# wwhitecyan/satellite-pose-estimation

Measured on AMD Instinct MI355X. Metric: images/sec end-to-end (backbone->kpts->PnP) at 416x416; SPEED pose score, higher is better.
Workload: dtype bf16; 1 GPU; BASELINE config 2: ResNet50-s8 + 6/6 DETR, 11 queries, 416x416, solver=epnp; global_batch=64, per_gpu_batch=64, input_size=416, num_queries=11, attention_dtype=bf16 q/k, fp16 V/P, parallelism=dp1 (image sharding)

## Files before the change

include/spe.h:

```cpp
#ifndef SPE_H_
#define SPE_H_
#include <stdint.h>

#ifdef __cplusplus
extern "C" {
#endif

#define SPE_ABI_VERSION 9

enum {
  SPE_E_ARG = -1,
  SPE_E_STATE = -2,
  SPE_E_MISSING = -3,
  SPE_E_KEY = -4,
  SPE_E_WORKSPACE = -5,
  SPE_E_LAUNCH = -6
};

enum { SPE_DTYPE_BF16_ = 0, SPE_DTYPE_F32_ = 1, SPE_DTYPE_F16_ = 2, SPE_DTYPE_F32X3_ = 4, SPE_DTYPE_F32X6_ = 5,
       SPE_DTYPE_F32H3_ = 6 };

enum { SPE_PNP_EPNP = 0, SPE_PNP_RANSAC_P3P_LM = 1, SPE_PNP_EPNP_RANSAC_SIGMA = 2, SPE_PNP_EPNP_LM = 3,
       SPE_PNP_EPNP_CERES = 4, SPE_PNP_EXHAUSTIVE = 5 };

// ... 153 lines not shown
                   int W, int Cin, int KH, int KW, int stride, int pad, const void* Bw, int ldb, int M, int N, int K,
                   const float* bias, const void* R, int ldr, int act_code, void* C, int ldc, int out_f32, int vt_T,
                   int vt_B, int r_period, const float* ln_g, const float* ln_b, int out_f16);
int spe_debug_gemm_path(void);
int spe_debug_gemm_h3(void* stream, int mode, const void* A, int lda, int H, int W, int Cin, int KH, int KW, int stride,
                      int pad, int ldb, int M, int N, int K, const float* bias, const void* R, int ldr, int act_code,
                      void* C, int ldc, const void* planes, int plane_rows, const float* sinv, const float* amax_a,
                      float* amax_c, float amax_c_mul);
int spe_debug_ffn_h3(void* stream, const float* x, int ldx, float* y, int ldy, int M, int F, const void* w1, int ld1,
                     const float* meta1, const void* w2, int ld2, const float* sinv2, const float* b2,
                     const float* gamma, const float* beta, const float* amax_x, float sh);
int spe_debug_ffn_h3_perm(int p);
int spe_debug_gemm_planes(void* stream, int dtype, int mode, const void* A, int lda, const void* P, int ldp, int prow,
                          int H, int W, int Cin, int KH, int KW, int stride, int pad, const void* Bw, int ldb, int M,
                          int N, int K, const float* bias, const void* R, int ldr, int act_code, void* C, int ldc,
                          const void* planes, int plane_rows);
int spe_debug_attention(void* stream, int dtype, const void* q, int ldq, const void* k, int ldk, const void* vt,
                        void* o, int ldo, int B, int H, int Tq, int Tk, float scale);
int spe_debug_attn_map(void* stream, const void* q, const void* k, int B, int H, int Tq, int Tk, int dtype, float* out);
int spe_debug_layernorm(void* stream, int dtype, const void* x, const float* gamma, const float* beta, void* out,
                        float* out_f32, int M, int D);
int spe_debug_ffn(void* stream, const void* x, int ldx, const void* w1, int ld1, const float* b1, const void* w2,
                  int ld2, const float* b2, const float* gamma, const float* beta, void* y, int ldy, int M, int D,
                  int F, float* partial, int splits);
int spe_debug_xattn(void* stream, const void* q, int ldq, const void* k, int ldk, const void* v, int ldv, void* u,
                    int ldu, const void* wv, const float* bv, void* o, int ldo, int B, int Q, int T, int splits,
                    float* partial_scratch);
int spe_debug_xattn_h3(void* stream, const float* q, int ldq, const float* mem, const float* pos, const float* mem_amax,
                       const float* wv, const float* bv, float* o, int ldo, float* o_amax, int B, int Q, int T,
                       int splits, float* partial_scratch, void* plane_scratch);
int spe_debug_upconv(void* stream, int dtype, const void* z, void* out, int ldo, int B, int H, int W, int C);
int spe_debug_btail(void* stream, const void* a, int lda, int k1, const void* r, const void* w3, int ld3,
                    const float* b3, void* y, const void* w1p, int ld1, const float* b1, void* z, int n2, int M);
int spe_debug_decsa(void* stream, void* tgt, int ldt, int B, int Q, const void* wqk, int ldqk, const float* bqk,
                    const void* wv, int ldv, const float* bv, const void* qpos, const void* wo, int ldo,
                    const float* bo, const float* g, const float* b, float scale);
int spe_debug_decproj(void* stream, void* tgt, int ldt, const void* x, int ldx, int B, int Q, const void* wo, int ldo,
                      const float* bo, const float* g, const float* b);
int spe_debug_decxproj(void* stream, void* tgt, int ldt, float* partial_scratch, int splits, int T, int B, int Q,
                       const void* wv, int ldwv, const float* bv, const void* wo, int ldo, const float* bo,
                       const float* g, const float* b);
int spe_debug_wfrag_pack(void* stream, const void* w, int ld, int N, void* dst);
int spe_debug_decffn(void* stream, const void* x, int ldx, int M, int F, const void* w1, int ld1, const float* b1,
                     const void* w2, int ld2, const float* b2, const float* gamma, const float* beta, void* y, int ldy,
                     float* partial);
int spe_debug_decq(void* stream, const void* x, int ldx, int M, int N, const void* w, int ldw, const float* bias,
                   const void* r, int ldr, int period, void* y, int ldy);
int spe_debug_btail_perm(int k);
int spe_debug_stempool(void* stream, const void* x, const void* w, int ldw, const float* bias, void* out, int ldo,
                       int B, int S);

int spe_debug_dwconv_tiles(int Ho, int Wo);
int spe_debug_dwconv(void* stream, int dtype, const void* x, const float* w, const float* bias, void* y,
                     float* pool_partials, int B, int H, int W, int C, int k, int stride, int act);
int spe_debug_se_gate(void* stream, const float* pool_partials, int tiles, float inv_hw, const float* w1, const float* b1,
                      const float* w2t, float* scale, int B, int C, int hidden);
int spe_debug_pwconv(void* stream, int dtype, const void* a, int lda, const void* w, int ldw, const float* bias,
                     const float* scale, int rows_per_image, const void* r, int ldr, void* c, int ldc, int M, int N,
                     int K, int act);
int spe_debug_rtdetr_backbone(spe_model* m, void* stream, const float* images, int batch, void* workspace,
                              int64_t workspace_bytes, float* f0, float* f1, float* f2);

int spe_debug_ghost_cheap(void* stream, int dtype, const void* x1, int ldx, int xoff, const float* w, const float* bias,
                          void* y, const void* gate, const void* resid, float* pool_partials, int B, int H, int W,
                          int half, int act, int post);
int spe_debug_dfc_gate(void* stream, int dtype, const void* x, const float* w1, const float* b1, const float* w2,
                       const float* b2, void* gate, int B, int H, int W, int C);
int spe_debug_se_gate_bias(void* stream, const float* pool_partials, int tiles, float inv_hw, const float* w1,
                           const float* b1, const float* w2t, const float* b2, float* scale, int B, int C, int hidden);
int spe_debug_pool2(void* stream, int dtype, const void* x, void* y, int B, int H, int W, int C);

int spe_debug_rt_resample2x(void* stream, int dtype, const void* in, int ldi, void* out, int ldo, int B, int H, int W,
                            int C, int mode);
int spe_debug_rt_query_select(void* stream, int dtype, const float* logits, int C, const void* memory, int ldm,
                              const float* anchors, int B, int Q, int D, int levels, const int* lvl_start, int* topk,
                              void* target, int ldt, float* sel_logits, float* sel_anchors);
int spe_debug_rt_qpos_hidden(void* stream, int dtype, const float* ref, const float* w0, const float* b0, void* out,
                             int rows, int H);
int spe_debug_rt_head_finish(void* stream, int dtype, int rows, int Q, int C, const float* hs, const float* cls_w,
                             const float* cls_b, const void* h2, int ld_h2, const float* box_w2, const float* box_b2,
                             const float* sig_w2, const float* sig_b2, const float* pt_add, int pt_add_invsig,
// ... 11 lines not shown
```

satellite-pose-estimation_amd/csrc/debug_capi.cpp:

```cpp
#include <hip/hip_runtime.h>

#include <cmath>

#include "../../include/spe.h"
#include "model_state.h"

namespace {
thread_local const void* g_planes = nullptr;
thread_local int g_plane_rows = 0;
}

extern "C" {

int spe_debug_gemm(void* stream, int dtype, int mode, const void* A, int lda, const void* P, int ldp, int prow,
                   int H, int W, int Cin, int KH, int KW, int stride, int pad, const void* Bw, int ldb, int M, int N,
                   int K, const float* bias, const void* R, int ldr, int act_code, void* C, int ldc, int out_f32, int vt_T,
                   int vt_B, int r_period, const float* ln_g, const float* ln_b, int out_f16) {
  GemmArgs g{};
  g.A = A; g.lda = lda; g.P = P; g.ldp = ldp; g.prow = prow;
  g.H = H; g.W = W; g.Cin = Cin; g.KH = KH; g.KW = KW; g.stride = stride; g.pad = pad;
  g.Ho = mode == GEMM_CONV ? (H + 2 * pad - KH) / stride + 1 : 0;
  g.Wo = mode == GEMM_CONV ? (W + 2 * pad - KW) / stride + 1 : 0;
  g.B = Bw; g.ldb = ldb; g.M = M; g.N = N; g.K = K;
  g.bias = bias; g.R = R; g.ldr = ldr; g.act = act_code & 255; g.res_post = (act_code >> 8) & 1; g.C = C; g.ldc = ldc; g.out_f32 = out_f32;
// ... 132 lines not shown
int spe_debug_xattn_h3(void* stream, const float* q, int ldq, const float* mem, const float* pos, const float* mem_amax,
                       const float* wv, const float* bv, float* o, int ldo, float* o_amax, int B, int Q, int T,
                       int splits, float* partial_scratch, void* plane_scratch) {
  if (!q || !mem || !pos || !mem_amax || !wv || !bv || !o || !partial_scratch || !plane_scratch || B < 0 || Q < 1 ||
      T < 1)
    return spe_fail(SPE_E_ARG, "bad argument");
  hipStream_t s = (hipStream_t)stream;
  char* kp = (char*)plane_scratch;
  char* vp = kp + (size_t)B * T * 1024;
  if (spe_launch_xattn_h3_split(mem, pos, mem_amax, kp, vp, B, T, s) != 0)
    return spe_fail(SPE_E_LAUNCH, "xattn_h3 split launch failed");
  XattnArgs a{};
  a.q = q; a.ldq = ldq; a.k = kp; a.ldk = 512; a.v = vp; a.ldv = 512;
  a.wv = wv; a.bv = bv; a.o = o; a.ldo = ldo;
  a.B = B; a.Q = Q; a.T = T; a.splits = splits > 0 ? splits : spe_xattn_splits(B, Q, T);
  const size_t rows = (size_t)a.splits * B * 8 * Q;
  a.pm = partial_scratch; a.pl = partial_scratch + rows; a.pu = partial_scratch + 2 * rows;
  a.mem_amax = mem_amax; a.o_amax = o_amax;
  const int rc = spe_launch_xattn_h3(a, s);
  return rc != 0 ? spe_fail(SPE_E_LAUNCH, "xattn_h3 launch rejected its arguments") : 0;
}

int spe_debug_btail(void* stream, const void* a, int lda, int k1, const void* r, const void* w3, int ld3,
                    const float* b3, void* y, const void* w1p, int ld1, const float* b1, void* z, int n2, int M) {
  if (!a || !w3 || !b3 || !y || !w1p || !b1 || !z || M < 0) return spe_fail(SPE_E_ARG, "bad argument");
  BtailArgs t{};
  t.A = a; t.lda = lda; t.k1 = k1; t.R = r; t.ldr = 256;
  t.w3 = w3; t.ld3 = ld3; t.b3 = b3; t.y = y; t.ldy = 256; t.n1 = 256;
  t.w1 = w1p; t.ld1 = ld1; t.b1 = b1; t.z = z; t.ldz = n2; t.n2 = n2; t.M = M;
  const int rc = spe_launch_btail(t, (hipStream_t)stream);
  return rc != 0 ? spe_fail(SPE_E_LAUNCH, "btail launch rejected its arguments") : 0;
}

namespace {
struct Frags {
  std::vector<void*> bufs;
  hipStream_t s;
  int err = 0;
  explicit Frags(hipStream_t st) : s(st) {}
  const void* get(const void* w, int ld, int N) {
    if (ld == 0 || !w) return w;
    void* p = nullptr;
    if (hipMalloc(&p, (size_t)N * 256 * 2) != hipSuccess) { err = 1; return nullptr; }
    bufs.push_back(p);
    if (spe_launch_wfrag_pack(w, ld, N, p, s) != 0) err = 1;
    return p;
  }
  ~Frags() {
    if (bufs.empty()) return;
    (void)hipStreamSynchronize(s);
    for (void* p : bufs) (void)hipFree(p);
  }
};
}

int spe_debug_wfrag_pack(void* stream, const void* w, int ld, int N, void* dst) {
  const int rc = spe_launch_wfrag_pack(w, ld, N, dst, (hipStream_t)stream);
  return rc != 0 ? spe_fail(SPE_E_ARG, "wfrag_pack: bad argument") : 0;
}

int spe_debug_decsa(void* stream, void* tgt, int ldt, int B, int Q, const void* wqk, int ldqk, const float* bqk,
                    const void* wv, int ldv, const float* bv, const void* qpos, const void* wo, int ldo,
                    const float* bo, const float* g, const float* b, float scale) {
  Frags f((hipStream_t)stream);
  DecSaArgs a{};
  a.tgt = tgt; a.ldt = ldt; a.B = B; a.Q = Q;
// ... 44 lines not shown
    a.w2 = w2;
  } else {
    void* p = nullptr;
    if (hipMalloc(&p, (size_t)256 * F * 2) != hipSuccess) return spe_fail(SPE_E_ARG, "decffn: scratch");
    f.bufs.push_back(p);
    for (int c0 = 0; c0 < F; c0 += 256)
      if (spe_launch_wfrag_pack((const char*)w2 + (size_t)c0 * 2, ld2, 256, (char*)p + (size_t)c0 * 256 * 2,
                                (hipStream_t)stream))
        f.err = 1;
    a.w2 = p;
  }
  if (f.err) return spe_fail(SPE_E_ARG, "decffn: weight packing failed");
  FfnArgs r{};
  r.x = x; r.ldx = ldx; r.y = y; r.ldy = ldy; r.M = M; r.D = 256; r.F = F;
  r.b2 = b2; r.gamma = gamma; r.beta = beta; r.splits = F / 256; r.partial = partial;
  int rc = spe_launch_decffn(a, (hipStream_t)stream);
  if (!rc) rc = spe_launch_ffn_reduce_ln(r, (hipStream_t)stream);
  return rc != 0 ? spe_fail(SPE_E_LAUNCH, "decffn launch rejected its arguments") : 0;
}

int spe_debug_decq(void* stream, const void* x, int ldx, int M, int N, const void* w, int ldw, const float* bias,
                   const void* r, int ldr, int period, void* y, int ldy) {
  if (!x || !w || !y || M < 0 || N < 256 || N % 256) return spe_fail(SPE_E_ARG, "bad argument");
  Frags f((hipStream_t)stream);
  DecQArgs a{};
  a.x = x; a.ldx = ldx; a.M = M; a.N = N; a.w = f.get(w, ldw, N); a.bias = bias;
  a.R = r; a.ldr = ldr; a.period = period; a.y = y; a.ldy = ldy;
  if (f.err) return spe_fail(SPE_E_ARG, "decq: weight packing failed");
  const int rc = spe_launch_decq(a, (hipStream_t)stream);
  return rc != 0 ? spe_fail(SPE_E_LAUNCH, "decq launch rejected its arguments") : 0;
}

int spe_debug_btail_perm(int k) { return spe_btail_perm(k); }

int spe_debug_stempool(void* stream, const void* x, const void* w, int ldw, const float* bias, void* out, int ldo,
                       int B, int S) {
  if (!x || !w || !bias || !out || B < 0) return spe_fail(SPE_E_ARG, "bad argument");
  const int rc = spe_launch_stempool(x, w, ldw, bias, out, ldo, B, S, (hipStream_t)stream);
  return rc != 0 ? spe_fail(SPE_E_LAUNCH, "stempool launch rejected its arguments") : 0;
}

int spe_debug_dwconv_tiles(int Ho, int Wo) { return Ho > 0 && Wo > 0 ? spe_mb_dwconv_tiles(Ho, Wo) : 0; }

int spe_debug_dwconv(void* stream, int dtype, const void* x, const float* w, const float* bias, void* y,
                     float* pool_partials, int B, int H, int W, int C, int k, int stride, int act) {
  if (!x || !w || !bias || !y) return spe_fail(SPE_E_ARG, "null argument");
  if (dtype != SPE_DTYPE_BF16 && dtype != SPE_DTYPE_F32) return spe_fail(SPE_E_ARG, "bad dtype");
  if (!spe_mb_dwconv_fits(B, H, W, C, k, stride) || (act != MB_ACT_NONE && act != MB_ACT_RELU && act != MB_ACT_HSWISH))
    return spe_fail(SPE_E_ARG, "dwconv: k must be 3 or 5, stride 1 or 2 (even H and W), C a multiple of 8, act 0 / 1 / 4");
  MbDwArgs a{};
  a.in = x; a.out = y; a.w = w; a.bias = bias; a.pool = pool_partials;
  a.B = B; a.H = H; a.W = W; a.C = C; a.k = k; a.stride = stride; a.act = act;
  const int rc = spe_launch_mb_dwconv(a, dtype, (hipStream_t)stream);
  return rc < 0 ? spe_fail(SPE_E_LAUNCH, "dwconv launch rejected its arguments") : rc;
}

int spe_debug_se_gate(void* stream, const float* pool_partials, int tiles, float inv_hw, const float* w1, const float* b1,
                      const float* w2t, float* scale, int B, int C, int hidden) {
  MbSeArgs a{};
  a.pool = pool_partials; a.tiles = tiles; a.inv_hw = inv_hw;
  a.w1 = w1; a.b1 = b1; a.w2t = w2t; a.scale = scale;
  a.B = B; a.C = C; a.hidden = hidden;
  const int rc = spe_launch_mb_se_gate(a, (hipStream_t)stream);
  return rc < 0 ? spe_fail(SPE_E_ARG, "se_gate: null argument, C > 1024 or hidden > 256") : rc;
}

// ... 134 lines not shown
```

satellite-pose-estimation_amd/csrc/forward.cpp:

```cpp
#include <hip/hip_runtime.h>

#include <cmath>

#include "launch.h"
#include "model_state.h"
#include "spe_common.h"

#define fail spe_fail
#define TRY(x)                         \
  do {                                 \
    if (const int _r = (x)) return _r; \
  } while (0)

namespace {

struct AttnTap {
  int enc_layer, dec_layer;
  float *enc_map, *dec_map;
};

struct Fwd {
  spe_model* m;
  Ws w;
  char* ws;
// ... 28 lines not shown
  return 0;
}

int unfused_ffn(Fwd& f, const char* kind1, const char* kind2, const char* ln_kind, const Conv& l1, const Conv& l2,
                void* x, const float* x_amax, int M, void* hidden, float* h_amax, void* tmp, const float* lg,
                const float* lb) {
  GemmArgs g = linear_args(l1, x, f.d, M, hidden, f.ff);
  g.act = ACT_RELU;
  g.amax_a = x_amax; g.amax_c = h_amax;
  CK(run_gemm(f.m, kind1, g, GEMM_LINEAR, f.s));
  return linear_residual_ln(f, kind2, ln_kind, l2, hidden, f.ff, h_amax, M, x, tmp, lg, lb);
}


struct BlockIn {
  size_t x;
  int ld, H;
  const float* amax;
  bool t1_ready;
};

int conv3_tail_or_gemm(Fwd& f, const Block* nb, const Conv& c3, const void* A, int lda, const float* a_amax,
                       const void* R, void* out, float* out_amax, int M, bool* tailed) {
  spe_model* m = f.m;
  int rc = 1;
  if (nb) {
    BtailArgs t{};
    t.A = A; t.lda = lda; t.k1 = c3.K; t.R = R; t.ldr = c3.N;
    t.w3 = c3.w; t.ld3 = c3.Kpad; t.b3 = c3.bias; t.y = out; t.ldy = c3.N; t.n1 = c3.N;
    t.w1 = nb->c1p.w; t.ld1 = nb->c1p.Kpad; t.b1 = nb->c1p.bias; t.z = f.P(f.w.t1); t.ldz = nb->c1.N; t.n2 = nb->c1.N;
    t.M = M;
    const double flops = 2.0 * M * ((double)c3.N * c3.K + (double)nb->c1.N * c3.N);
    const double bytes = ((double)M * (c3.K + c3.N + nb->c1.N) + (R ? (double)M * c3.N : 0.0)) * m->esz;
    rc = run_other(m, "conv.1x1", flops, bytes, f.s, [&] { return spe_launch_btail(t, f.s); });
    if (rc != 0 && rc != 1) CK(rc);
  }
  if (rc == 1) {
    GemmArgs g = linear_args(c3, A, lda, M, out, c3.N);
    if (R) { g.R = R; g.ldr = c3.N; }
    g.act = ACT_RELU;
    g.amax_a = a_amax; g.amax_c = out_amax;
    CK(run_gemm(m, "conv.1x1", g, GEMM_LINEAR, f.s));
  }
  *tailed = rc == 0;
  return 0;
}

int bottleneck(Fwd& f, size_t bi, BlockIn& in) {
  spe_model* m = f.m;
  const Ws& w = f.w;
  hipStream_t s = f.s;
  const int B = f.B, H = in.H;
  const Block& blk = m->blocks[bi];
  const bool fused = bi == 0 && blk.c3ds.w != nullptr;
  const Block* nb = bi + 1 < m->blocks.size() && m->blocks[bi + 1].c1p.w ? &m->blocks[bi + 1] : nullptr;
  const size_t outbuf = (bi == 6) ? w.xs8 : (in.x == w.bufA ? w.bufB : w.bufA);
  const int Ho = (H + 2 - 3) / blk.stride + 1;
  float* const t1_amax = f.slot(2 + 3 * (int)bi);
  float* const t2_amax = f.slot(2 + 3 * (int)bi + 1);
  float* const out_amax = f.slot(2 + 3 * (int)bi + 2);
  if (!in.t1_ready) {
    GemmArgs g = linear_args(blk.c1, f.P(in.x), in.ld, B * H * H, f.P(w.t1), blk.c1.N);
    g.act = ACT_RELU;
    g.amax_a = in.amax; g.amax_c = t1_amax;
    CK(run_gemm(m, "conv.1x1", g, GEMM_LINEAR, s));
  }
  {
// ... 601 lines not shown
```

satellite-pose-estimation_amd/csrc/registry.cpp:

```cpp
#include <hip/hip_runtime.h>

#include <algorithm>
#include <cmath>
#include <cstdlib>
#include <cstdio>
#include <cstring>

#include "model_state.h"
#include "registry.h"

namespace {
thread_local std::string g_err;
}

uint16_t f2bf(float f) {
  uint32_t u;
  std::memcpy(&u, &f, 4);
  if ((u & 0x7fffffffu) > 0x7f800000u) return (uint16_t)((u >> 16) | 0x40);
  u += 0x7fffu + ((u >> 16) & 1u);
  return (uint16_t)(u >> 16);
}

int spe_fail(int code, const std::string& msg) {
  g_err = msg;
// ... 403 lines not shown
  m->blocks.clear();
  const int nblk[3] = {3, 4, 6};
  for (int li = 0; li < 3; ++li)
    for (int k = 0; k < nblk[li]; ++k) {
      std::string p = b + ".layer" + std::to_string(li + 1) + "." + std::to_string(k);
      Block blk;
      blk.stride = (k == 0 && li > 0) ? 2 : 1;
      blk.c1 = make_conv(m, p + ".conv1.weight", p + ".bn1", "", 0, 1, 0);
      blk.c2 = make_conv(m, p + ".conv2.weight", p + ".bn2", "", 0, blk.stride, 1);
      blk.c3 = make_conv(m, p + ".conv3.weight", p + ".bn3", "", 0, 1, 0);
      if (k == 0) {
        blk.has_ds = true;
        blk.ds = make_conv(m, p + ".downsample.0.weight", p + ".downsample.1", "", 0, blk.stride, 0);
        if (blk.stride == 1 && m->esz == 2) {
          std::vector<float> w3, b3, wd, bd;
          fold_conv(m, p + ".conv3.weight", p + ".bn3", "", w3, b3);
          fold_conv(m, p + ".downsample.0.weight", p + ".downsample.1", "", wd, bd);
          const int n = blk.c3.N, k3 = blk.c3.K, kd = blk.ds.K;
          std::vector<float> rows((size_t)n * (k3 + kd));
          if (m->dmem)
            for (int r = 0; r < n; ++r) {
              for (int c = 0; c < k3; ++c) rows[(size_t)r * (k3 + kd) + c] = w3[(size_t)r * k3 + c];
              for (int c = 0; c < kd; ++c) rows[(size_t)r * (k3 + kd) + k3 + c] = wd[(size_t)r * kd + c];
            }
          std::vector<float> bias(n);
          for (int r = 0; r < n; ++r) bias[r] = b3[r] + bd[r];
          Conv& f = blk.c3ds;
          f.N = n; f.K = k3 + kd; f.Kpad = pad64(f.K); f.Cin = f.K;
          f.w = upload_rows(m, rows, f.N, f.K, f.Kpad);
          f.bias = upload_f32(m, bias.data(), bias.size());
        }
      }
      const int gi = li == 0 ? k : (li == 1 && k == 0 ? 3 : -1);
      if (m->esz == 2 && spe_btail_enabled() && gi >= 1 && blk.c1.K == 256) {
        std::vector<float> w1, b1;
        fold_conv(m, p + ".conv1.weight", p + ".bn1", "", w1, b1);
        const int n = blk.c1.N, K = blk.c1.K;
        std::vector<float> rows((size_t)n * K, 0.f);
        if (m->dmem)
          for (int r = 0; r < n; ++r)
            for (int c = 0; c < K; ++c) rows[(size_t)r * K + c] = w1[(size_t)r * K + spe_btail_perm(c)];
        Conv& f = blk.c1p;
        f.N = n; f.K = K; f.Kpad = pad64(K); f.Cin = K;
        f.w = upload_rows(m, rows, f.N, f.K, f.Kpad);
        f.bias = upload_f32(m, b1.data(), b1.size());
      }
      m->blocks.push_back(blk);
    }
  m->s8 = make_conv(m, "backbone.0.s8_latern.weight", "", "", 0, 1, 0);
  m->s16 = make_conv(m, "backbone.0.s16_latern.weight", "", "", 0, 1, 1);
  m->s16taps = Conv{};
  if (spe_use_upconv(m)) {
    const auto sh = param_shape(m, "backbone.0.s16_latern.weight");
    const int co_n = (int)sh[0], ci_n = (int)sh[1];
    std::vector<float> rows;
    if (m->dmem) {
      const auto& src = m->host["backbone.0.s16_latern.weight"];
      rows.assign((size_t)9 * co_n * ci_n, 0.f);
      for (int t = 0; t < 9; ++t)
        for (int co = 0; co < co_n; ++co)
          for (int ci = 0; ci < ci_n; ++ci)
            rows[((size_t)t * co_n + co) * ci_n + ci] = src[((size_t)co * ci_n + ci) * 9 + t];
    }
    Conv& c = m->s16taps;
    c.N = 9 * co_n; c.K = ci_n; c.Kpad = pad64(ci_n); c.Cin = ci_n;
    c.w = upload_rows(m, rows, c.N, c.K, c.Kpad);
  }
  m->outc = make_conv(m, "backbone.0.output_conv.weight", "", "backbone.0.output_conv.bias", 0, 1, 1);
  m->inproj = make_conv(m, "input_proj.weight", "", "input_proj.bias", 0, 1, 0);
  m->neckip = Conv{};
  if (spe_use_neckfold(m)) {
    const auto so = param_shape(m, "backbone.0.output_conv.weight");
    const auto sp = param_shape(m, "input_proj.weight");
    const int cm = (int)so[0], ci_n = (int)so[1], co_n = (int)sp[0], taps = (int)(so[2] * so[3]);
// ... 299 lines not shown
```

satellite-pose-estimation_amd/csrc/spe_kernels.h:

```cpp
#pragma once
#include <hip/hip_runtime.h>
#include <stdint.h>

enum { SPE_DTYPE_BF16 = 0, SPE_DTYPE_F32 = 1, SPE_DTYPE_F16 = 2,
       SPE_DTYPE_BF16_F16V = 3,
       SPE_DTYPE_F32X3 = 4,
       SPE_DTYPE_F32X6 = 5,
       SPE_DTYPE_F32H3 = 6 };
enum { GEMM_LINEAR = 0, GEMM_LINEAR_ADD = 1, GEMM_CONV = 2 };
enum { ACT_NONE = 0, ACT_RELU = 1, ACT_SILU = 2, ACT_GELU = 3 };

struct GemmArgs {
  const void* A; int lda;
  const void* P; int ldp; int prow;
  int H, W, Cin, KH, KW, stride, pad, Ho, Wo;
  const void* B; int ldb;
  int M, N, K;
  const float* bias;
  const void* R; int ldr;
  int act;
  int res_post;
  void* C; int ldc;
  int out_f32;
  int out_f16;
// ... 8 lines not shown
  float* amax_c; float amax_c_mul;
  int s_f16; float s_l1, s_bmax;
};
bool spe_gemm_ln_fusable(const GemmArgs& g);
int spe_launch_gemm(const GemmArgs& g, int dtype, int mode, hipStream_t s);
int spe_launch_gemm_h3(const GemmArgs& g, int mode, hipStream_t s);

__host__ __device__ inline bool conv_channel_blocked(int Cin, int taps) { return (Cin & 63) == 0 && taps > 1; }
__device__ __forceinline__ void conv_k_decode(int k, int Cin, int KW, int taps, int& kh, int& kw, int& ci) {
  int tap;
  if (conv_channel_blocked(Cin, taps)) {
    const int cb = k / (64 * taps), rem = k - cb * 64 * taps;
    tap = rem >> 6;
    ci = cb * 64 + (rem & 63);
  } else {
    tap = k / Cin;
    ci = k - tap * Cin;
  }
  kh = tap / KW;
  kw = tap - kh * KW;
}
struct BtailArgs {
  const void* A; int lda; int k1;
  const void* R; int ldr;
  const void* w3; int ld3; const float* b3;
  void* y; int ldy; int n1;
  const void* w1; int ld1; const float* b1;
  void* z; int ldz; int n2;
  int M;
};
int spe_launch_btail(const BtailArgs& a, hipStream_t s);
int spe_btail_perm(int k);
bool spe_btail_enabled();
int spe_launch_gemm2(const GemmArgs& g, int mode, hipStream_t s);
int spe_launch_sgemm(const GemmArgs& g, int mode, hipStream_t s);
int spe_launch_lnproj(const GemmArgs& g, hipStream_t s);
bool spe_lnproj_applies(const GemmArgs& g);
inline bool spe_ln_fusable(const GemmArgs& g) { return spe_lnproj_applies(g) || spe_gemm_ln_fusable(g); }
int spe_launch_pconv(const GemmArgs& g, hipStream_t s);
int spe_cu_count();
extern thread_local int spe_gemm_last_path;

__host__ __device__ inline int vt_pos(int t) { return (t & ~12) | ((t & 4) << 1) | ((t & 8) >> 1); }

struct AttnArgs {
  const void* q; int ldq;
  const void* k; int ldk;
  const void* vt;
  int vt_swz;
  void* o; int ldo;
  int B, H, Tq, Tk;
  float scale;
  int presplit;
  int v_f16;
  const float* v_amax; float v_l1, v_bmax;
};
int spe_launch_attention_split(const AttnArgs& a, hipStream_t s);
int spe_launch_attention(const AttnArgs& a, int dtype, hipStream_t s);

struct AttnMapArgs {
  const void* q; long long q_sb, q_sh; int ldq;
  const void* k; long long k_sb, k_sh; int ldk;
  float* out;
  int B, H, Tq, Tk;
  int head_dim;
  float scale;
// ... 281 lines not shown
```

satellite-pose-estimation_amd/spe/_lib.py:

```python
from __future__ import annotations

import ctypes
import os

import torch

if os.environ.get("SPE_GRAPH_CAPTURE") == "1":
    os.environ.setdefault("DEBUG_CLR_GRAPH_PACKET_CAPTURE", "0")

_HERE = os.path.dirname(os.path.abspath(__file__))
LIB_PATH = os.environ.get("SPE_LIB_PATH") or os.path.join(_HERE, "libspe.so")

ABI_VERSION = 9

P = ctypes.c_void_p
I = ctypes.c_int
I64 = ctypes.c_int64
F = ctypes.c_float
D = ctypes.c_double

SPE_DTYPE_BF16, SPE_DTYPE_F32, SPE_DTYPE_F16, SPE_DTYPE_F32X3, SPE_DTYPE_F32X6, SPE_DTYPE_F32H3 = 0, 1, 2, 4, 5, 6
SPE_RTDETR_MBV3_LARGE = 1003
SPE_RTDETR_GHOSTNETV2 = 1004
GH_POST_NONE, GH_POST_GATE, GH_POST_RESIDUAL = 0, 1, 2
MB_ACT_NONE, MB_ACT_RELU, MB_ACT_HSWISH = 0, 1, 4
SPE_STAGE_ENCODE, SPE_STAGE_DECODE, SPE_STAGE_BACKBONE, SPE_STAGE_TRANSFORMER = 1, 2, 4, 8
SPE_PNP_EPNP, SPE_PNP_RANSAC_P3P_LM, SPE_PNP_EPNP_RANSAC_SIGMA, SPE_PNP_EPNP_LM, SPE_PNP_EPNP_CERES = 0, 1, 2, 3, 4
SPE_PNP_EXHAUSTIVE = 5
SPE_PNP_OK, SPE_PNP_NO_FG, SPE_PNP_CV_ERROR, SPE_PNP_RANSAC_FALLBACK, SPE_PNP_UNPINNED = 0, 1, 2, 3, 4

EXPORTS = ["spe_abi_version", "spe_last_error", "spe_model_create", "spe_model_destroy", "spe_model_set_param",
           "spe_model_num_params", "spe_model_param_name", "spe_model_finalize", "spe_model_workspace_bytes",
           "spe_forward", "spe_forward_stages", "spe_forward_stages_u8", "spe_preprocess", "spe_preprocess_submission", "spe_criterion", "spe_criterion_sigma", "spe_ensemble_fuse", "spe_postprocess", "spe_pnp_batch", "spe_pnp_exhaustive", "spe_debug_pnp_exhaustive_stages", "spe_self_assess", "spe_speed_score", "spe_model_profile_begin",
           "spe_model_profile_end", "spe_model_profile_get", "spe_debug_gemm", "spe_debug_gemm_path", "spe_debug_gemm_h3", "spe_debug_ffn_h3", "spe_debug_ffn_h3_perm", "spe_debug_gemm_planes", "spe_debug_attention",
           "spe_debug_layernorm", "spe_debug_ffn", "spe_debug_xattn", "spe_debug_xattn_h3", "spe_debug_upconv", "spe_debug_btail", "spe_debug_decsa", "spe_debug_decproj", "spe_debug_decxproj", "spe_debug_wfrag_pack", "spe_debug_decffn", "spe_debug_decq", "spe_debug_btail_perm", "spe_debug_stempool", "spe_rtdetr_create", "spe_rtdetr_forward",
           "spe_rtdetr_forward_stages", "spe_rtdetr_forward_stages_u8",
           "spe_jpeg_workspace_bytes", "spe_jpeg_decode",
           "spe_debug_dwconv_tiles", "spe_debug_dwconv", "spe_debug_se_gate", "spe_debug_pwconv", "spe_debug_rtdetr_backbone",
           "spe_debug_ghost_cheap", "spe_debug_dfc_gate", "spe_debug_se_gate_bias", "spe_debug_pool2",
           "spe_debug_rt_resample2x", "spe_debug_rt_query_select", "spe_debug_rt_qpos_hidden", "spe_debug_rt_head_finish",
           "spe_debug_rt_msdeform",
           "spe_forward_attention", "spe_forward_attention_workspace_bytes", "spe_debug_attn_map"]


class ModelConfig(ctypes.Structure):
    _fields_ = [("input_size", I), ("num_queries", I), ("enc_layers", I), ("dec_layers", I), ("hidden_dim", I),
                ("nheads", I), ("dim_feedforward", I), ("sigma_head", I), ("dtype", I),
                ("attn_dtype", I)]


class ForwardOutputs(ctypes.Structure):
    _fields_ = [("logits", P), ("points", P), ("clip_bbox", P), ("probs", P), ("points_px", P),
                ("log_sigmas", P), ("sigmas", P), ("hs", P), ("aux_logits", P), ("aux_points", P)]


class RtdetrConfig(ctypes.Structure):
    _fields_ = [("depth", I), ("input_size", I), ("num_queries", I), ("dec_layers", I), ("enc_ff", I), ("dec_ff", I),
                ("csp_hidden", I), ("num_classes", I), ("dtype", I)]


class RtdetrOutputs(ctypes.Structure):
    _fields_ = [("logits", P), ("points", P), ("log_sigmas", P), ("clip_bbox", P), ("probs", P), ("points_px", P),
                ("sigmas", P), ("aux_logits", P), ("aux_points", P), ("aux_log_sigmas", P), ("enc_logits", P),
                ("enc_points", P), ("topk", P), ("hs", P)]


class SpeError(RuntimeError):
    pass
# ... 29 lines not shown
    L.spe_forward_attention.argtypes = [P, P, P, I, P, I64, ctypes.POINTER(ForwardOutputs), I, I, P, P]
    L.spe_forward_attention_workspace_bytes.argtypes = [P, I]
    L.spe_forward_attention_workspace_bytes.restype = I64
    L.spe_debug_attn_map.argtypes = [P, P, P, I, I, I, I, I, P]
    L.spe_postprocess.argtypes = [P, P, P, P, I, I, P, P]
    L.spe_preprocess.argtypes = [P, P, I, I, I, I, P, I, P, P, P]
    L.spe_preprocess_submission.argtypes = [P, P, I, I, I, I, P, I, P, P, P, P]
    L.spe_ensemble_fuse.argtypes = [P, P, P, I, I, I, I, P, P]
    L.spe_criterion.argtypes = [P, P, P, P, P, I, I, I, I, I, F, F, F, D, P, P]
    L.spe_criterion_sigma.argtypes = [P, P, P, P, P, P, P, I, I, I, I, I, F, F, I, F, D, P, P]
    L.spe_pnp_batch.argtypes = [P, P, P, P, I, I, I, P, P, I, F, I, D, P, P, P, P, P, P, P, P]
    L.spe_pnp_exhaustive.argtypes = [P, P, P, P, I, I, I, P, P, F, I, P, P, P, P, P, P, P, P, P, P]
    L.spe_debug_pnp_exhaustive_stages.argtypes = L.spe_pnp_exhaustive.argtypes + [I]
    L.spe_speed_score.argtypes = [P, P, P, P, P, I, P, P]
    L.spe_self_assess.argtypes = [P, P, P, P, P, P, I, I, I, F, F, I, P, P, P]
    L.spe_model_profile_begin.argtypes = [P, ctypes.c_char_p]
    L.spe_model_profile_end.argtypes = [P]
    L.spe_model_profile_get.argtypes = [P, I, ctypes.c_char_p, I, ctypes.POINTER(D), ctypes.POINTER(D),
                                        ctypes.POINTER(D)]
    L.spe_debug_gemm.argtypes = [P, I, I, P, I, P, I, I] + [I] * 7 + [P, I, I, I, I, P, P, I, I, P, I, I, I, I, I, P, P, I]
    L.spe_debug_gemm_path.argtypes = []
    L.spe_debug_gemm_h3.argtypes = [P, I, P, I] + [I] * 7 + [I, I, I, I, P, P, I, I, P, I, P, I, P, P, P, ctypes.c_float]
    L.spe_debug_ffn_h3.argtypes = [P, P, I, P, I, I, I, P, I, P, P, I, P, P, P, P, P, ctypes.c_float]
    L.spe_debug_ffn_h3_perm.argtypes = [I]
    L.spe_debug_gemm_planes.argtypes = [P, I, I, P, I, P, I, I] + [I] * 7 + [P, I, I, I, I, P, P, I, I, P, I, P, I]
    L.spe_debug_attention.argtypes = [P, I, P, I, P, I, P, P, I, I, I, I, I, F]
    L.spe_debug_layernorm.argtypes = [P, I, P, P, P, P, P, I, I]
    L.spe_debug_ffn.argtypes = [P, P, I, P, I, P, P, I, P, P, P, P, I, I, I, I, P, I]
    L.spe_debug_xattn.argtypes = [P, P, I, P, I, P, I, P, I, P, P, P, I, I, I, I, I, P]
    L.spe_debug_xattn_h3.argtypes = [P, P, I, P, P, P, P, P, P, I, P, I, I, I, I, P, P]
    L.spe_debug_upconv.argtypes = [P, I, P, P, I, I, I, I, I]
    L.spe_debug_btail.argtypes = [P, P, I, I, P, P, I, P, P, P, I, P, P, I, I]
    L.spe_debug_btail_perm.argtypes = [I]
    L.spe_debug_decsa.argtypes = [P, P, I, I, I, P, I, P, P, I, P, P, P, I, P, P, P, ctypes.c_float]
    L.spe_debug_decproj.argtypes = [P, P, I, P, I, I, I, P, I, P, P, P]
    L.spe_debug_wfrag_pack.argtypes = [P, P, I, I, P]
    L.spe_debug_decffn.argtypes = [P, P, I, I, I, P, I, P, P, I, P, P, P, P, I, P]
    L.spe_debug_decq.argtypes = [P, P, I, I, I, P, I, P, P, I, I, P, I]
    L.spe_debug_decxproj.argtypes = [P, P, I, P, I, I, I, I, P, I, P, P, I, P, P, P]
    L.spe_debug_stempool.argtypes = [P, P, P, I, P, P, I, I, I]
    L.spe_rtdetr_create.argtypes = [ctypes.POINTER(RtdetrConfig), ctypes.POINTER(P)]
    L.spe_rtdetr_forward.argtypes = [P, P, P, I, P, I64, ctypes.POINTER(RtdetrOutputs)]
    L.spe_rtdetr_forward_stages.argtypes = [P, P, P, I, P, I64, ctypes.POINTER(RtdetrOutputs), I]
    L.spe_rtdetr_forward_stages_u8.argtypes = [P, P, P, I, I, P, I64, ctypes.POINTER(RtdetrOutputs), I]
    L.spe_debug_dwconv_tiles.argtypes = [I, I]
    L.spe_debug_dwconv.argtypes = [P, I, P, P, P, P, P, I, I, I, I, I, I, I]
    L.spe_debug_se_gate.argtypes = [P, P, I, F, P, P, P, P, I, I, I]
    L.spe_debug_pwconv.argtypes = [P, I, P, I, P, I, P, P, I, P, I, P, I, I, I, I, I]
    L.spe_debug_rtdetr_backbone.argtypes = [P, P, P, I, P, I64, P, P, P]
    L.spe_debug_ghost_cheap.argtypes = [P, I, P, I, I, P, P, P, P, P, P, I, I, I, I, I, I]
    L.spe_debug_dfc_gate.argtypes = [P, I, P, P, P, P, P, P, I, I, I, I]
    L.spe_debug_se_gate_bias.argtypes = [P, P, I, F, P, P, P, P, P, I, I, I]
    L.spe_debug_pool2.argtypes = [P, I, P, P, I, I, I, I]
    IP = ctypes.POINTER(I)
    L.spe_debug_rt_resample2x.argtypes = [P, I, P, I, P, I, I, I, I, I, I]
    L.spe_debug_rt_query_select.argtypes = [P, I, P, I, P, I, P, I, I, I, I, IP, P, P, I, P, P]
    L.spe_debug_rt_qpos_hidden.argtypes = [P, I, P, P, P, P, I, I]
    L.spe_debug_rt_head_finish.argtypes = [P, I, I, I, I, P, P, P, P, I, P, P, P, P, P, I, P, P, P, P, P, P, P]
    L.spe_debug_rt_msdeform.argtypes = [P, I, P, I, P, I, P, P, I, I, I, I, I, I, IP, IP, IP]
    L.spe_jpeg_workspace_bytes.argtypes = [I, I, I, I64]
    L.spe_jpeg_workspace_bytes.restype = I64
    L.spe_jpeg_decode.argtypes = [P, P, P, P, I, I, I, I64, P, P, P, I64]
    return L


def lib():
# ... 22 lines not shown
```

Measured before the change: 6017 images/s.

## Add wide bottleneck-tail fused kernel for 512/1024-channel ResNet stages

Adds a fused kernel that computes a bottleneck block's conv3 (with bias, residual and ReLU) and the next block's conv1 in one pass for the wider ResNet stages (n1=512 or 1024). The intermediate activation stays in registers for the second MFMA GEMM, so it does not have to be read back from memory. Weights are streamed through a 3-stage LDS pipeline using buffer-to-LDS loads. Folded conv1 weights are uploaded for these blocks, and the forward pass picks the new path when enough tiles exist to fill half the CUs. The trade-off is that tile counts drop, so per-CU work grows and occupancy may be limited by LDS and register use.

```diff
diff --git a/include/spe.h b/include/spe.h
--- a/include/spe.h
+++ b/include/spe.h
@@ -209,6 +209,9 @@
 int spe_debug_upconv(void* stream, int dtype, const void* z, void* out, int ldo, int B, int H, int W, int C);
 int spe_debug_btail(void* stream, const void* a, int lda, int k1, const void* r, const void* w3, int ld3,
                     const float* b3, void* y, const void* w1p, int ld1, const float* b1, void* z, int n2, int M);
+int spe_debug_btail_wide(void* stream, const void* a, int lda, int k1, const void* r, int ldr, const void* w3, int ld3,
+                         const float* b3, void* y, int ldy, int n1, const void* w1p, int ld1, const float* b1, void* z,
+                         int ldz, int n2, int M);
 int spe_debug_decsa(void* stream, void* tgt, int ldt, int B, int Q, const void* wqk, int ldqk, const float* bqk,
                     const void* wv, int ldv, const float* bv, const void* qpos, const void* wo, int ldo,
                     const float* bo, const float* g, const float* b, float scale);
@@ -224,6 +227,7 @@
 int spe_debug_decq(void* stream, const void* x, int ldx, int M, int N, const void* w, int ldw, const float* bias,
                    const void* r, int ldr, int period, void* y, int ldy);
 int spe_debug_btail_perm(int k);
+int spe_debug_btail_wide_perm(int n1, int k);
 int spe_debug_stempool(void* stream, const void* x, const void* w, int ldw, const float* bias, void* out, int ldo,
                        int B, int S);
 
diff --git a/satellite-pose-estimation_amd/csrc/btail_wide.hip b/satellite-pose-estimation_amd/csrc/btail_wide.hip
--- /dev/null
+++ b/satellite-pose-estimation_amd/csrc/btail_wide.hip
@@ -0,0 +1,243 @@
+#include "spe_common.h"
+#include "spe_kernels.h"
+
+#include <algorithm>
+#include <cstdlib>
+
+namespace {
+
+typedef __attribute__((address_space(3))) void* lds_ptr_t;
+constexpr int NT = 256, HC = 32, NST = 3;
+constexpr int BAD = 0x7ffffff0;
+constexpr int N1MAX = 1024;
+
+template <int N>
+SPE_DEV void wait_vmcnt() { asm volatile("s_waitcnt vmcnt(%0)" ::"n"(N) : "memory"); }
+
+SPE_DEV int w3_src_row(int r) { return 8 * ((r & 15) >> 2) + 4 * (r >> 4) + (r & 3); }
+SPE_DEV int w1_key(int n) { return (4 - ((n >> 2) & 3)) & 3; }
+SPE_DEV int w1_off(int n, int c) { return n * 64 + ((c ^ w1_key(n)) << 4); }
+
+template <int K1, int N2, int MB, bool HAS_R>
+struct WideDma {
+  static constexpr int KB1 = K1 * 2;
+  static constexpr int W3_BYTES = HC * KB1, W1_BYTES = N2 * HC * 2;
+  static constexpr int L3 = W3_BYTES / 1024 / 4, L1 = W1_BYTES / 1024 / 4;
+  static constexpr int RPI = 1024 / KB1, LPR = KB1 / 16;
+  __amdgpu_buffer_rsrc_t r3, r1, rr;
+  int vo3[L3], vo1[L1], vor[MB];
+  SPE_DEV void init(const BtailArgs& a, int m0, int wid, int lane) {
+    r3 = __builtin_amdgcn_make_buffer_rsrc((void*)a.w3, (short)0, a.n1 * a.ld3 * 2, 0x00020000);
+    r1 = __builtin_amdgcn_make_buffer_rsrc((void*)a.w1, (short)0, N2 * a.ld1 * 2, 0x00020000);
+    rr = __builtin_amdgcn_make_buffer_rsrc((void*)a.R, (short)0, HAS_R ? ((a.M - 1) * a.ldr + a.n1) * 2 : 0, 0x00020000);
+#pragma unroll
+    for (int i = 0; i < L3; ++i) {
+      const int r = RPI * (wid * L3 + i) + lane / LPR, c = (lane % LPR) ^ (r & 15);
+      vo3[i] = (w3_src_row(r) * a.ld3 + c * 8) * 2;
+    }
+#pragma unroll
+    for (int i = 0; i < L1; ++i) {
+      const int n = 16 * (wid * L1 + i) + (lane >> 2), c = (lane & 3) ^ w1_key(n);
+      vo1[i] = (n * a.ld1 + c * 8) * 2;
+    }
+#pragma unroll
+    for (int mb = 0; mb < MB; ++mb) {
+      const int m = m0 + 16 * mb + (lane & 15);
+      vor[mb] = m < a.M ? (m * a.ldr + 8 * (lane >> 4)) * 2 : BAD;
+    }
+  }
+  SPE_DEV void issue(const BtailArgs& a, int ch, char* st, int wid) const {
+#pragma unroll
+    for (int i = 0; i < L3; ++i)
+      __builtin_amdgcn_raw_ptr_buffer_load_lds(r3, (lds_ptr_t)(st + (wid * L3 + i) * 1024), 16, vo3[i], ch * HC * a.ld3 * 2, 0, 0);
+#pragma unroll
+    for (int i = 0; i < L1; ++i)
+      __builtin_amdgcn_raw_ptr_buffer_load_lds(r1, (lds_ptr_t)(st + W3_BYTES + (wid * L1 + i) * 1024), 16, vo1[i], ch * HC * 2, 0, 0);
+    if constexpr (HAS_R) {
+#pragma unroll
+      for (int mb = 0; mb < MB; ++mb)
+        __builtin_amdgcn_raw_ptr_buffer_load_lds(rr, (lds_ptr_t)(st + W3_BYTES + W1_BYTES + (wid * MB + mb) * 1024), 16, vor[mb],
+                                                 ch * HC * 2, 0, 0);
+    }
+  }
+};
+
+template <int K1, int N2, int MB, bool HAS_R>
+__global__ __launch_bounds__(NT, (N2 == 128 && MB <= 2) ? 2 : 1) void btail_wide_kernel(BtailArgs a) {
+  constexpr int KB1 = K1 * 2, KF1 = K1 / 32, NB2 = N2 / 16;
+  constexpr int W3_BYTES = HC * KB1, W1_BYTES = N2 * HC * 2, R_BYTES = HAS_R ? 4 * MB * 1024 : 0;
+  constexpr int STAGE = W3_BYTES + W1_BYTES + R_BYTES;
+  constexpr int L3 = W3_BYTES / 1024 / 4, L1 = W1_BYTES / 1024 / 4;
+  constexpr int LOADS = L3 + L1 + (HAS_R ? MB : 0);
+  __shared__ __attribute__((aligned(1024))) char lds[NST * STAGE + (N1MAX + N2) * 4];
+  float* sb3 = reinterpret_cast<float*>(lds + NST * STAGE);
+  float* sb1 = sb3 + N1MAX;
+  const int tid = threadIdx.x, lane = tid & 63, wid = __builtin_amdgcn_readfirstlane(tid >> 6);
+  const int g = lane >> 4, c16 = lane & 15;
+  const int m0 = blockIdx.x * 64 * MB + wid * 16 * MB;
+  const int nch = a.n1 / HC;
+  for (int i = tid; i < a.n1; i += NT) sb3[i] = a.b3[i];
+  for (int i = tid; i < N2; i += NT) sb1[i] = a.b1[i];
+
+  bf16x8 xf[MB][KF1];
+#pragma unroll
+  for (int mb = 0; mb < MB; ++mb) {
+    const int m = m0 + 16 * mb + c16;
+    const bf16* xr = (const bf16*)a.A + (size_t)(m < a.M ? m : 0) * a.lda;
+#pragma unroll
+    for (int ks = 0; ks < KF1; ++ks)
+      xf[mb][ks] = __builtin_bit_cast(bf16x8, m < a.M ? ld16(xr + 32 * ks + 8 * g) : u32x4{0, 0, 0, 0});
+  }
+  f32x4 acc[NB2][MB];
+#pragma unroll
+  for (int nb = 0; nb < NB2; ++nb)
+#pragma unroll
+    for (int mb = 0; mb < MB; ++mb) acc[nb][mb] = f32x4{0, 0, 0, 0};
+
+  const __amdgpu_buffer_rsrc_t ry =
+      __builtin_amdgcn_make_buffer_rsrc(a.y, (short)0, ((a.M - 1) * a.ldy + a.n1) * 2, 0x00020000);
+  int voy[MB];
+#pragma unroll
+  for (int mb = 0; mb < MB; ++mb) {
+    const int m = m0 + 16 * mb + c16;
+    voy[mb] = m < a.M ? (m * a.ldy + 8 * g) * 2 : BAD;
+  }
+  WideDma<K1, N2, MB, HAS_R> dma;
+  dma.init(a, m0, wid, lane);
+
+#pragma unroll
+  for (int mb = 0; mb < MB; ++mb)
+#pragma unroll
+    for (int ks = 0; ks < KF1; ++ks) asm volatile("" ::"v"(xf[mb][ks]));
+  wait_vmcnt<0>();
+  dma.issue(a, 0, lds, wid);
+  dma.issue(a, 1, lds + STAGE, wid);
+
+  int slot = 0;
+  for (int ch = 0; ch < nch; ++ch) {
+    if (ch == 0) wait_vmcnt<LOADS>();
+    else if (ch + 1 < nch) wait_vmcnt<LOADS + MB>();
+    else wait_vmcnt<MB>();
+    asm volatile("s_waitcnt lgkmcnt(0)" ::: "memory");
+    __builtin_amdgcn_s_barrier();
+    const int slot2 = slot == 0 ? NST - 1 : slot - 1;
+    const char* st = lds + slot * STAGE;
+    slot = slot == NST - 1 ? 0 : slot + 1;
+    u32x4 wa[KF1][2], wb[NB2], rv[HAS_R ? MB : 1];
+#pragma unroll
+    for (int ks = 0; ks < KF1; ++ks)
+#pragma unroll
+      for (int jb = 0; jb < 2; ++jb) {
+        const int r = 16 * jb + c16;
+        wa[ks][jb] = ld16(st + r * KB1 + (((4 * ks + g) ^ (r & 15)) << 4));
+      }
+    if constexpr (HAS_R) {
+#pragma unroll
+      for (int mb = 0; mb < MB; ++mb) rv[mb] = ld16(st + W3_BYTES + W1_BYTES + (wid * MB + mb) * 1024 + lane * 16);
+    }
+#pragma unroll
+    for (int nb = 0; nb < NB2; ++nb) wb[nb] = ld16(st + W3_BYTES + w1_off(16 * nb + c16, g));
+    if (ch + 2 < nch) dma.issue(a, ch + 2, lds + slot2 * STAGE, wid);
+    __builtin_amdgcn_sched_barrier(0);
+    f32x4 h[2][MB];
+#pragma unroll
+    for (int jb = 0; jb < 2; ++jb)
+#pragma unroll
+      for (int mb = 0; mb < MB; ++mb) h[jb][mb] = f32x4{0, 0, 0, 0};
+#pragma unroll
+    for (int ks = 0; ks < KF1; ++ks)
+#pragma unroll
+      for (int jb = 0; jb < 2; ++jb) {
+        const bf16x8 w = __builtin_bit_cast(bf16x8, wa[ks][jb]);
+#pragma unroll
+        for (int mb = 0; mb < MB; ++mb)
+          h[jb][mb] = __builtin_amdgcn_mfma_f32_16x16x32_bf16(w, xf[mb][ks], h[jb][mb], 0, 0, 0);
+      }
+    const f32x4 b3a = *reinterpret_cast<const f32x4*>(sb3 + ch * HC + 8 * g);
+    const f32x4 b3b = *reinterpret_cast<const f32x4*>(sb3 + ch * HC + 8 * g + 4);
+    bf16x8 yb[MB];
+#pragma unroll
+    for (int mb = 0; mb < MB; ++mb) {
+      float v[8];
+#pragma unroll
+      for (int r = 0; r < 4; ++r) {
+        v[r] = h[0][mb][r] + b3a[r];
+        v[4 + r] = h[1][mb][r] + b3b[r];
+      }
+      if constexpr (HAS_R) {
+        float rf[8];
+        unpack16<bf16>(rv[mb], rf);
+#pragma unroll
+        for (int e = 0; e < 8; ++e) v[e] += rf[e];
+      }
+#pragma unroll
+      for (int e = 0; e < 8; ++e) v[e] = fmaxf(v[e], 0.f);
+      const u32x4 yw = pack16<bf16>(v);
+      __builtin_amdgcn_raw_buffer_store_b128(yw, ry, voy[mb], ch * HC * 2, 0);
+      yb[mb] = __builtin_bit_cast(bf16x8, yw);
+    }
+#pragma unroll
+    for (int nb = 0; nb < NB2; ++nb) {
+      const bf16x8 w = __builtin_bit_cast(bf16x8, wb[nb]);
+#pragma unroll
+      for (int mb = 0; mb < MB; ++mb)
+        acc[nb][mb] = __builtin_amdgcn_mfma_f32_16x16x32_bf16(w, yb[mb], acc[nb][mb], 0, 0, 0);
+    }
+  }
+
+#pragma unroll
+  for (int mb = 0; mb < MB; ++mb) {
+    const int m = m0 + 16 * mb + c16;
+    if (m >= a.M) continue;
+    bf16* zr = (bf16*)a.z + (size_t)m * a.ldz;
+#pragma unroll
+    for (int nb = 0; nb < NB2; ++nb) {
+      const int n = 16 * nb + 4 * g;
+      const f32x4 bv = *reinterpret_cast<const f32x4*>(sb1 + n);
+      float v[4];
+#pragma unroll
+      for (int r = 0; r < 4; ++r) v[r] = fmaxf(acc[nb][mb][r] + bv[r], 0.f);
+      st8(zr + n, u32x2{pack_bf16x2(v[0], v[1]), pack_bf16x2(v[2], v[3])});
+    }
+  }
+}
+
+template <int K1, int N2, int MB>
+int launch(const BtailArgs& a, hipStream_t s) {
+  const int tiles = (a.M + 64 * MB - 1) / (64 * MB);
+  if (a.R) hipLaunchKernelGGL((btail_wide_kernel<K1, N2, MB, true>), dim3(tiles), dim3(NT), 0, s, a);
+  else hipLaunchKernelGGL((btail_wide_kernel<K1, N2, MB, false>), dim3(tiles), dim3(NT), 0, s, a);
+  return (int)hipGetLastError();
+}
+
+}
+
+int spe_btail_wide_perm(int n1, int k) { return k >= 0 && k < n1 ? k : -1; }
+
+bool spe_btail_wide_enabled() {
+  static const int on = spe_env_int("SPE_BTAIL_WIDE", 1);
+  return on != 0;
+}
+
+namespace {
+int tile_rows(const BtailArgs& a) { return a.n1 == 1024 ? 192 : 128; }
+}
+
+int spe_btail_wide_tiles(const BtailArgs& a) { return (a.M + tile_rows(a) - 1) / tile_rows(a); }
+
+bool spe_btail_wide_serves(const BtailArgs& a) {
+  if (!spe_btail_wide_enabled()) return false;
+  if (a.lda % 8 || a.ldy % 8 || a.ldz % 4 || (a.R && a.ldr % 8) || a.lda < a.k1 || a.ldy < a.n1 || a.ldz < a.n2 ||
+      (a.R && a.ldr < a.n1) || a.ld3 < a.k1 || a.ld1 < a.n1 || a.ld3 % 8 || a.ld1 % 8)
+    return false;
+  if ((double)a.M * std::max(a.ldy, a.R ? a.ldr : 0) * 2 >= 2147483648.0) return false;
+  return (a.k1 == 128 && a.n1 == 512 && (a.n2 == 128 || a.n2 == 256)) || (a.k1 == 256 && a.n1 == 1024 && a.n2 == 256);
+}
+
+int spe_launch_btail_wide(const BtailArgs& a, hipStream_t s) {
+  if (a.M <= 0) return 0;
+  if (!spe_btail_wide_serves(a)) return 1;
+  if (a.n1 == 1024) return launch<256, 256, 3>(a, s);
+  if (a.n2 == 128) return launch<128, 128, 2>(a, s);
+  return launch<128, 256, 2>(a, s);
+}
diff --git a/satellite-pose-estimation_amd/csrc/debug_capi.cpp b/satellite-pose-estimation_amd/csrc/debug_capi.cpp
--- a/satellite-pose-estimation_amd/csrc/debug_capi.cpp
+++ b/satellite-pose-estimation_amd/csrc/debug_capi.cpp
@@ -188,6 +188,18 @@
   return rc != 0 ? spe_fail(SPE_E_LAUNCH, "btail launch rejected its arguments") : 0;
 }
 
+int spe_debug_btail_wide(void* stream, const void* a, int lda, int k1, const void* r, int ldr, const void* w3, int ld3,
+                         const float* b3, void* y, int ldy, int n1, const void* w1p, int ld1, const float* b1, void* z,
+                         int ldz, int n2, int M) {
+  if (!a || !w3 || !b3 || !y || !w1p || !b1 || !z || M < 0) return spe_fail(SPE_E_ARG, "bad argument");
+  BtailArgs t{};
+  t.A = a; t.lda = lda; t.k1 = k1; t.R = r; t.ldr = ldr;
+  t.w3 = w3; t.ld3 = ld3; t.b3 = b3; t.y = y; t.ldy = ldy; t.n1 = n1;
+  t.w1 = w1p; t.ld1 = ld1; t.b1 = b1; t.z = z; t.ldz = ldz; t.n2 = n2; t.M = M;
+  const int rc = spe_launch_btail_wide(t, (hipStream_t)stream);
+  return rc != 0 && rc != 1 ? spe_fail(SPE_E_LAUNCH, "btail_wide launch failed") : rc;
+}
+
 namespace {
 struct Frags {
   std::vector<void*> bufs;
@@ -298,6 +310,7 @@
 }
 
 int spe_debug_btail_perm(int k) { return spe_btail_perm(k); }
+int spe_debug_btail_wide_perm(int n1, int k) { return spe_btail_wide_perm(n1, k); }
 
 int spe_debug_stempool(void* stream, const void* x, const void* w, int ldw, const float* bias, void* out, int ldo,
                        int B, int S) {
diff --git a/satellite-pose-estimation_amd/csrc/forward.cpp b/satellite-pose-estimation_amd/csrc/forward.cpp
--- a/satellite-pose-estimation_amd/csrc/forward.cpp
+++ b/satellite-pose-estimation_amd/csrc/forward.cpp
@@ -84,7 +84,11 @@
     t.M = M;
     const double flops = 2.0 * M * ((double)c3.N * c3.K + (double)nb->c1.N * c3.N);
     const double bytes = ((double)M * (c3.K + c3.N + nb->c1.N) + (R ? (double)M * c3.N : 0.0)) * m->esz;
-    rc = run_other(m, "conv.1x1", flops, bytes, f.s, [&] { return spe_launch_btail(t, f.s); });
+    if (c3.N == 256) {
+      rc = run_other(m, "conv.1x1", flops, bytes, f.s, [&] { return spe_launch_btail(t, f.s); });
+    } else if (spe_btail_wide_serves(t) && spe_btail_wide_tiles(t) >= spe_cu_count() / 2) {
+      rc = run_other(m, "conv.1x1", flops, bytes, f.s, [&] { return spe_launch_btail_wide(t, f.s); });
+    }
     if (rc != 0 && rc != 1) CK(rc);
   }
   if (rc == 1) {
diff --git a/satellite-pose-estimation_amd/csrc/registry.cpp b/satellite-pose-estimation_amd/csrc/registry.cpp
--- a/satellite-pose-estimation_amd/csrc/registry.cpp
+++ b/satellite-pose-estimation_amd/csrc/registry.cpp
@@ -459,14 +459,17 @@
         }
       }
       const int gi = li == 0 ? k : (li == 1 && k == 0 ? 3 : -1);
-      if (m->esz == 2 && spe_btail_enabled() && gi >= 1 && blk.c1.K == 256) {
+      const bool narrow = spe_btail_enabled() && gi >= 1 && blk.c1.K == 256;
+      const bool wide = spe_btail_wide_enabled() && li >= 1 && !m->blocks.empty() && m->blocks.back().c3.N == blk.c1.K &&
+                        (blk.c1.K == 512 || blk.c1.K == 1024);
+      if (m->esz == 2 && (narrow || wide)) {
         std::vector<float> w1, b1;
         fold_conv(m, p + ".conv1.weight", p + ".bn1", "", w1, b1);
         const int n = blk.c1.N, K = blk.c1.K;
         std::vector<float> rows((size_t)n * K, 0.f);
         if (m->dmem)
           for (int r = 0; r < n; ++r)
-            for (int c = 0; c < K; ++c) rows[(size_t)r * K + c] = w1[(size_t)r * K + spe_btail_perm(c)];
+            for (int c = 0; c < K; ++c) rows[(size_t)r * K + c] = w1[(size_t)r * K + (wide ? spe_btail_wide_perm(K, c) : spe_btail_perm(c))];
         Conv& f = blk.c1p;
         f.N = n; f.K = K; f.Kpad = pad64(K); f.Cin = K;
         f.w = upload_rows(m, rows, f.N, f.K, f.Kpad);
diff --git a/satellite-pose-estimation_amd/csrc/spe_kernels.h b/satellite-pose-estimation_amd/csrc/spe_kernels.h
--- a/satellite-pose-estimation_amd/csrc/spe_kernels.h
+++ b/satellite-pose-estimation_amd/csrc/spe_kernels.h
@@ -64,6 +64,11 @@
 int spe_launch_btail(const BtailArgs& a, hipStream_t s);
 int spe_btail_perm(int k);
 bool spe_btail_enabled();
+int spe_launch_btail_wide(const BtailArgs& a, hipStream_t s);
+int spe_btail_wide_perm(int n1, int k);
+bool spe_btail_wide_enabled();
+bool spe_btail_wide_serves(const BtailArgs& a);
+int spe_btail_wide_tiles(const BtailArgs& a);
 int spe_launch_gemm2(const GemmArgs& g, int mode, hipStream_t s);
 int spe_launch_sgemm(const GemmArgs& g, int mode, hipStream_t s);
 int spe_launch_lnproj(const GemmArgs& g, hipStream_t s);
diff --git a/satellite-pose-estimation_amd/spe/_lib.py b/satellite-pose-estimation_amd/spe/_lib.py
--- a/satellite-pose-estimation_amd/spe/_lib.py
+++ b/satellite-pose-estimation_amd/spe/_lib.py
@@ -33,7 +33,7 @@
            "spe_model_num_params", "spe_model_param_name", "spe_model_finalize", "spe_model_workspace_bytes",
            "spe_forward", "spe_forward_stages", "spe_forward_stages_u8", "spe_preprocess", "spe_preprocess_submission", "spe_criterion", "spe_criterion_sigma", "spe_ensemble_fuse", "spe_postprocess", "spe_pnp_batch", "spe_pnp_exhaustive", "spe_debug_pnp_exhaustive_stages", "spe_self_assess", "spe_speed_score", "spe_model_profile_begin",
            "spe_model_profile_end", "spe_model_profile_get", "spe_debug_gemm", "spe_debug_gemm_path", "spe_debug_gemm_h3", "spe_debug_ffn_h3", "spe_debug_ffn_h3_perm", "spe_debug_gemm_planes", "spe_debug_attention",
-           "spe_debug_layernorm", "spe_debug_ffn", "spe_debug_xattn", "spe_debug_xattn_h3", "spe_debug_upconv", "spe_debug_btail", "spe_debug_decsa", "spe_debug_decproj", "spe_debug_decxproj", "spe_debug_wfrag_pack", "spe_debug_decffn", "spe_debug_decq", "spe_debug_btail_perm", "spe_debug_stempool", "spe_rtdetr_create", "spe_rtdetr_forward",
+           "spe_debug_layernorm", "spe_debug_ffn", "spe_debug_xattn", "spe_debug_xattn_h3", "spe_debug_upconv", "spe_debug_btail", "spe_debug_decsa", "spe_debug_decproj", "spe_debug_decxproj", "spe_debug_wfrag_pack", "spe_debug_decffn", "spe_debug_decq", "spe_debug_btail_perm", "spe_debug_btail_wide", "spe_debug_btail_wide_perm", "spe_debug_stempool", "spe_rtdetr_create", "spe_rtdetr_forward",
            "spe_rtdetr_forward_stages", "spe_rtdetr_forward_stages_u8",
            "spe_jpeg_workspace_bytes", "spe_jpeg_decode",
            "spe_debug_dwconv_tiles", "spe_debug_dwconv", "spe_debug_se_gate", "spe_debug_pwconv", "spe_debug_rtdetr_backbone",
@@ -129,6 +129,8 @@
     L.spe_debug_upconv.argtypes = [P, I, P, P, I, I, I, I, I]
     L.spe_debug_btail.argtypes = [P, P, I, I, P, P, I, P, P, P, I, P, P, I, I]
     L.spe_debug_btail_perm.argtypes = [I]
+    L.spe_debug_btail_wide.argtypes = [P, P, I, I, P, I, P, I, P, P, I, I, P, I, P, P, I, I, I]
+    L.spe_debug_btail_wide_perm.argtypes = [I, I]
     L.spe_debug_decsa.argtypes = [P, P, I, I, I, P, I, P, P, I, P, P, P, I, P, P, P, ctypes.c_float]
     L.spe_debug_decproj.argtypes = [P, P, I, P, I, I, I, P, I, P, P, P]
     L.spe_debug_wfrag_pack.argtypes = [P, P, I, I, P]
```

Measured after the change: 6102 images/s, median of 6. 1.4% higher.
